# Symb0x76/ChineseChessZero

Hardware: NVIDIA B200
Metric: self-play moves/sec at 400 playouts (higher is better)
Workload: dtype bf16

## Files before the change

### chinesechesszero_b200/_lib.py

```python
from __future__ import annotations

import ctypes
import os

import numpy as np
import torch

from . import build as _build

BOARD_BYTES = 96
MAX_MOVES = 128
N_ACTIONS = 2086
PLANE_ELEMS = 10710
KEY_WINDOW = 128

FLAG_CHECK, FLAG_NOMOVES, FLAG_INSUFFICIENT, FLAG_FOURFOLD, FLAG_SIXTY = 1, 2, 4, 8, 16
FLAG_TIE_MASK = FLAG_INSUFFICIENT | FLAG_FOURFOLD | FLAG_SIXTY
STATUS_EXPAND_FAILED, STATUS_TREE_DROPPED = 1, 2
STATUS_NODE_OVERFLOW = STATUS_EXPAND_FAILED
ADVANCE_NEW_GAME, ADVANCE_DROP_TREE, ADVANCE_KEEP = -1, -2, -3
CTL_HEAD, CTL_TAIL, CTL_EXPAND_FAILED, CTL_TREES_DROPPED, CTL_MIN_FREE, CTL_WORDS = 0, 1, 2, 3, 4, 8
NODE_BYTES = 24
MAX_CHILDREN = 119
POLICY_PROBS, POLICY_LOGITS = 0, 1
CONV_VARIANT_1CTA, CONV_VARIANT_PAIR, CONV_VARIANT_2PAIRS, CONV_VARIANT_4PAIRS = 1, 2, 2 | 32, 2 | 64

EXPORTS = (
    "ccz_version", "ccz_last_error", "ccz_init", "ccz_action_table", "ccz_set_order_policy", "ccz_get_order_policy",
    "ccz_boards_start",
    "ccz_movegen_encode", "ccz_board_keys_init", "ccz_board_push", "ccz_mcts_pool_init", "ccz_mcts_reset",
    "ccz_mcts_reserve", "ccz_mcts_migrate", "ccz_mcts_select",
    "ccz_mcts_expand_backup", "ccz_mcts_root_visits", "ccz_mcts_advance", "ccz_replay_pack", "ccz_conv3x3_c256", "ccz_conv3x3_plan", "ccz_stem_lookup",
    "ccz_heads_pack",
)


class CczError(RuntimeError):
    pass


class ArenaStruct(ctypes.Structure):

    _fields_ = [
        ("n_games", ctypes.c_int32),
        ("n_pages", ctypes.c_int32),
        ("page_shift", ctypes.c_int32),
        ("max_pages", ctypes.c_int32),
        ("d_nodes", ctypes.c_void_p),
        ("d_links", ctypes.c_void_p),
        ("d_free_ring", ctypes.c_void_p),
        ("d_pool_ctl", ctypes.c_void_p),
        ("d_page_list", ctypes.c_void_p),
        ("d_page_fill", ctypes.c_void_p),
        ("d_n_pages", ctypes.c_void_p),
        ("d_n_pages_new", ctypes.c_void_p),
        ("d_list_sel", ctypes.c_void_p),
        ("d_alloc_page", ctypes.c_void_p),
        ("d_alloc_off", ctypes.c_void_p),
        ("d_root", ctypes.c_void_p),
        ("d_n_nodes", ctypes.c_void_p),
        ("d_status", ctypes.c_void_p),
        ("d_root_boards", ctypes.c_void_p),
        ("d_root_keys", ctypes.c_void_p),
    ]


# ... 15 lines not shown
        except Exception as e:
            if not os.path.exists(path):
                raise CczError(f"building {path} failed ({e}); there is no CPU fallback") from e
    if not os.path.exists(path):
        raise CczError(
            f"{path} is missing: run `python -c 'import __graft_entry__ as g; g.build()'` "
            "(nvcc -gencode arch=compute_100a,code=sm_100a); there is no CPU fallback"
        )
    lib = ctypes.CDLL(path)
    vp, i32, f32 = ctypes.c_void_p, ctypes.c_int, ctypes.c_float
    lib.ccz_version.restype = i32
    lib.ccz_last_error.restype = ctypes.c_char_p
    lib.ccz_init.restype = i32
    lib.ccz_action_table.argtypes = [vp, vp, vp]
    lib.ccz_boards_start.argtypes = [vp, i32, vp]
    lib.ccz_set_order_policy.argtypes = [vp]
    lib.ccz_get_order_policy.argtypes = [vp]
    lib.ccz_movegen_encode.argtypes = [vp, i32, vp, vp, vp, vp, vp]
    lib.ccz_board_keys_init.argtypes = [vp, i32, vp, vp]
    lib.ccz_board_push.argtypes = [vp, vp, i32, vp, vp]
    lib.ccz_mcts_pool_init.argtypes = [ctypes.POINTER(ArenaStruct), vp]
    lib.ccz_mcts_reset.argtypes = [ctypes.POINTER(ArenaStruct), vp, vp]
    lib.ccz_mcts_reserve.argtypes = [ctypes.POINTER(ArenaStruct), i32, vp]
    lib.ccz_mcts_migrate.argtypes = [ctypes.POINTER(ArenaStruct), ctypes.POINTER(ArenaStruct), vp]
    lib.ccz_mcts_select.argtypes = [ctypes.POINTER(ArenaStruct), f32, vp, vp, vp]
    lib.ccz_mcts_expand_backup.argtypes = [ctypes.POINTER(ArenaStruct), vp, vp, i32, vp, vp, vp, vp, vp]
    lib.ccz_mcts_root_visits.argtypes = [ctypes.POINTER(ArenaStruct), vp, vp, vp, vp]
    lib.ccz_mcts_advance.argtypes = [ctypes.POINTER(ArenaStruct), vp, vp]
    lib.ccz_replay_pack.argtypes = [vp, vp, vp, vp, vp, i32, vp, vp, vp]
    lib.ccz_conv3x3_c256.argtypes = [vp, vp, vp, vp, vp, i32, i32, vp]
    lib.ccz_stem_lookup.argtypes = [vp, i32, vp, vp, vp, vp]
    lib.ccz_conv3x3_plan.argtypes = [i32, i32, i32, vp]
    lib.ccz_heads_pack.argtypes = [vp, i32, vp, i32, i32, vp]
    for name in EXPORTS:
        if name not in ("ccz_last_error",):
            getattr(lib, name).restype = i32
    _lib = lib
    pinned = os.path.join(os.path.dirname(os.path.abspath(__file__)), "order_policy.json")
    if os.path.exists(pinned):
        import json

        with open(pinned) as f:
            set_order_policy(json.load(f))
    return lib


def check(rc: int, what: str) -> None:
    if rc != 0:
        msg = load().ccz_last_error().decode("utf-8", "replace")
        raise CczError(f"{what} failed ({rc}): {msg}")


def stream_ptr(device=None) -> int:
    return torch.cuda.current_stream(device).cuda_stream


def _ptr(t: torch.Tensor | None) -> int | None:
    if t is None:
        return None
    if not t.is_cuda:
        raise CczError("device tensor expected (the C ABI takes device pointers)")
    if not t.is_contiguous():
        raise CczError("contiguous tensor expected")
    return t.data_ptr()


# ... 240 lines not shown
                                    out.data_ptr(), int(x.shape[0]), int(variant), stream_ptr(x.device)),
            "ccz_conv3x3_c256",
        )
    return out


def stem_lookup(boards: torch.Tensor, table: torch.Tensor, bias_turn: torch.Tensor, out: torch.Tensor | None = None) -> torch.Tensor:
    n = boards.shape[0]
    if boards.dtype != torch.uint8 or boards.shape[1:] != (BOARD_BYTES,):
        raise CczError("stem_lookup: boards must be uint8 (n,96)")
    if table.dtype != torch.bfloat16 or tuple(table.shape) != (9, 16, 256) or bias_turn.dtype != torch.float32 \
            or tuple(bias_turn.shape) != (2, 9, 256):
        raise CczError("stem_lookup: table must be bf16 (9,16,256) and bias_turn fp32 (2,9,256)")
    if out is None:
        out = torch.empty((n, 256, 10, 9), dtype=torch.bfloat16, device=boards.device).contiguous(memory_format=torch.channels_last)
    elif tuple(out.shape) != (n, 256, 10, 9) or out.dtype != torch.bfloat16 or not out.is_contiguous(memory_format=torch.channels_last):
        raise CczError("stem_lookup: out must be bf16 (n,256,10,9) channels_last")
    with torch.cuda.device(boards.device):
        check(load().ccz_stem_lookup(_ptr(boards), n, _ptr(table), _ptr(bias_turn), out.data_ptr(), stream_ptr(boards.device)),
              "ccz_stem_lookup")
    return out


def heads_pack(h: torch.Tensor, operands: torch.Tensor, value_off: int) -> torch.Tensor:
    n = operands.shape[0]
    if h.dtype != torch.bfloat16 or operands.dtype != torch.bfloat16 or tuple(h.shape) != (n * 90, 32):
        raise CczError("heads_pack: h must be bf16 (n*90, 32) and operands bf16 (n, K)")
    with torch.cuda.device(h.device):
        check(load().ccz_heads_pack(_ptr(h), n, _ptr(operands), int(operands.shape[1]), int(value_off), stream_ptr(h.device)),
              "ccz_heads_pack")
    return operands


def conv3x3_plan(n_boards: int, variant: int = 0, resident_clusters: int = 74) -> dict:
    out = (ctypes.c_int32 * 6)()
    check(load().ccz_conv3x3_plan(int(n_boards), int(variant), int(resident_clusters), out), "ccz_conv3x3_plan")
    keys = ("rows_per_tile", "n_tiles", "n_items", "n_full", "split_log2", "clusters")
    return dict(zip(keys, (int(v) for v in out)))
```

### chinesechesszero_b200/csrc/ccz_b200.cu

```cuda
#include "../../include/ccz_b200.h"

#include <cuda_runtime.h>

#include <cstdio>
#include <cstdlib>
#include <cstring>
#include <utility>
#include <string>

#include "ccz_movegen.cuh"
#include "ccz_mcts.cuh"
#include "ccz_replay.cuh"
#include "ccz_conv.cuh"
#include "ccz_stem.cuh"
#include "ccz_heads.cuh"

#ifndef CCZ_CONV_DEFAULT_PAIRS
#define CCZ_CONV_DEFAULT_PAIRS 1
#endif

namespace {

thread_local std::string g_err;

// ... 439 lines not shown
            return fail(-3, "ccz_conv3x3_c256: cuTensorMapEncodeTiled(skip) failed");
    } else {
        ts = ty;
    }
    cudaError_t e;
#define CCZ_CONV_LAUNCH(CG, PAIRS)                                                                                      \
    (d_skip ? cv::launch_variant<CG, PAIRS, true>(tx, tw, ts, ty, d_bias, n_tiles, tail_split, dbg, s)     \
            : cv::launch_variant<CG, PAIRS, false>(tx, tw, ts, ty, d_bias, n_tiles, tail_split, dbg, s))
    if (cta_group == 1) e = CCZ_CONV_LAUNCH(1, 1);
    else if (pairs == 1) e = CCZ_CONV_LAUNCH(2, 1);
    else if (pairs == 2) e = CCZ_CONV_LAUNCH(2, 2);
    else e = CCZ_CONV_LAUNCH(2, 4);
#undef CCZ_CONV_LAUNCH
    if (e != cudaSuccess) return fail(-2, "conv3x3_c256_kernel launch", e);
    return 0;
}

int ccz_conv3x3_plan(int n_boards, int variant, int resident_clusters, int32_t *out) {
    namespace cv = ccz::conv;
    if (n_boards <= 0 || resident_clusters <= 0 || !out || variant < 0 || variant >= 128)
        return fail(-1, "ccz_conv3x3_plan: bad argument");
    int cta_group = variant & 3, pairs = 1 << ((variant >> 5) & 3);
    if (variant == 0) { cta_group = 2; pairs = CCZ_CONV_DEFAULT_PAIRS; }
    if (cta_group == 0) cta_group = 2;
    if (cta_group == 3 || pairs > 4 || (cta_group == 1 && pairs != 1)) return fail(-1, "ccz_conv3x3_plan: unsupported variant");
    const long long m = (long long)n_boards * cv::BOARD_HW;
    const int rows_per_tile = cv::BM * cta_group * pairs;
    const int n_tiles = (int)((m + rows_per_tile - 1) / rows_per_tile);
    const cv::Plan pl = cv::plan_items(n_tiles, resident_clusters, !(variant & 4));
    out[0] = rows_per_tile; out[1] = n_tiles; out[2] = pl.n_items; out[3] = pl.n_full; out[4] = pl.split_log2; out[5] = pl.clusters;
    return 0;
}

int ccz_stem_lookup(const uint8_t *d_boards, int n, const void *d_table, const float *d_bias_turn, void *d_y, ccz_stream_t s) {
    namespace st = ccz::stem;
    if (n < 0) return fail(-1, "ccz_stem_lookup: n < 0");
    if (n == 0) return 0;
    if (!d_boards || !d_table || !d_bias_turn || !d_y) return fail(-1, "ccz_stem_lookup: NULL pointer");
    if (((uintptr_t)d_boards & 3) || (((uintptr_t)d_table | (uintptr_t)d_bias_turn | (uintptr_t)d_y) & 15))
        return fail(-1, "ccz_stem_lookup: pointers must be 16-byte aligned (boards 4-byte)");
    static int n_sm_dev[64] = {0};
    int dev = 0;
    CCZ_CUDA(cudaGetDevice(&dev));
    if (dev < 0 || dev >= 64) return fail(-1, "ccz_stem_lookup: device index out of range");
    int &n_sm = n_sm_dev[dev];
    if (!n_sm) {
        CCZ_CUDA(cudaDeviceGetAttribute(&n_sm, cudaDevAttrMultiProcessorCount, dev));
        CCZ_CUDA(cudaFuncSetAttribute(st::stem_lookup_kernel, cudaFuncAttributeMaxDynamicSharedMemorySize, st::SMEM_BYTES));
    }
    int blocks = 2 * n_sm;
    const int need = (n + st::WARPS - 1) / st::WARPS;
    if (blocks > need) blocks = need;
    st::stem_lookup_kernel<<<blocks, st::WARPS * 32, st::SMEM_BYTES, s>>>(d_boards, n, static_cast<const uint4 *>(d_table),
                                                                         reinterpret_cast<const float4 *>(d_bias_turn),
                                                                         static_cast<uint4 *>(d_y));
    return check_launch("stem_lookup_kernel");
}

int ccz_heads_pack(const void *d_h, int n, void *d_operands, int row_elems, int value_off, ccz_stream_t s) {
    namespace hd = ccz::heads;
    if (n < 0) return fail(-1, "ccz_heads_pack: n < 0");
    if (n == 0) return 0;
    if (!d_h || !d_operands) return fail(-1, "ccz_heads_pack: NULL pointer");
    if (((uintptr_t)d_h & 15) || ((uintptr_t)d_operands & 3)) return fail(-1, "ccz_heads_pack: h must be 16-byte, operands 4-byte aligned");
    if ((row_elems & 1) || (value_off & 1) || value_off < hd::N_POLICY * hd::HW || row_elems < value_off + hd::N_VALUE * hd::HW)
        return fail(-1, "ccz_heads_pack: operand row must hold 1530 policy + 630 value elements at even offsets");
// ... 7 lines not shown
```

### chinesechesszero_b200/csrc/ccz_conv.cuh

```cuda
#pragma once

#include <cuda.h>
#include <cuda_bf16.h>
#include <cuda_runtime.h>

#include <cstdint>

#ifndef CCZ_CONV_BACKOFF_NS
#define CCZ_CONV_BACKOFF_NS 256
#endif

namespace ccz {
namespace conv {

constexpr int C = 256;
constexpr int BOARD_H = 10, BOARD_W = 9, BOARD_HW = 90;
constexpr int BM = 128;
constexpr int BN = 256;
constexpr int BK = 64;
constexpr int KBLOCKS = 9 * (C / BK);
constexpr int UMMA_K = 16;
constexpr int THREADS = 256;

template <int CG>
// ... 385 lines not shown
                    o.z = pack_bf16x2(fmaxf(f[4], 0.f), fmaxf(f[5], 0.f));
                    o.w = pack_bf16x2(fmaxf(f[6], 0.f), fmaxf(f[7], 0.f));
                    *cell = o;
                }
            }
            tc_fence_before();
            __syncwarp();
            if (lane == 0) {
                if constexpr (CG == 2) mbar_arrive_cluster(tempty0 + 8 * acc); else mbar_arrive(bar_tempty + 8 * acc);
            }
            if (++acc == 2) { acc = 0; acc_phase ^= 1; }
            fence_proxy_async();
            asm volatile("bar.sync 1, 128;" ::: "memory");
            if (threadIdx.x == 128) {
                for (int g = 0; g < wi.n_w / 64; ++g) tma_store_2d(&tm_y, staging + g * (BM * 128), wi.n_off + g * 64, m0);
                tma_store_commit();
                tma_store_wait_read();
                if (HAS_SKIP) mbar_arrive(bar_stfree);
            }
            asm volatile("bar.sync 1, 128;" ::: "memory");
        }
        if (threadIdx.x == 128) tma_store_wait_all();
    }

    __syncwarp();
    tc_fence_before();
    if constexpr (CLUSTER > 1) cluster_sync_all(); else __syncthreads();
    if (warp == 2) {
        tc_fence_after();
        tmem_dealloc<CG>(tmem_base, 512);
    }
}

typedef CUresult (*EncodeTiledFn)(CUtensorMap *, CUtensorMapDataType, cuuint32_t, void *, const cuuint64_t *, const cuuint64_t *,
                                  const cuuint32_t *, const cuuint32_t *, CUtensorMapInterleave, CUtensorMapSwizzle, CUtensorMapL2promotion,
                                  CUtensorMapFloatOOBfill);
typedef CUresult (*EncodeIm2colFn)(CUtensorMap *, CUtensorMapDataType, cuuint32_t, void *, const cuuint64_t *, const cuuint64_t *, const int *,
                                   const int *, cuuint32_t, cuuint32_t, const cuuint32_t *, CUtensorMapInterleave, CUtensorMapSwizzle,
                                   CUtensorMapL2promotion, CUtensorMapFloatOOBfill);

struct Driver {
    EncodeTiledFn tiled = nullptr;
    EncodeIm2colFn im2col = nullptr;
    bool ready = false;
};

inline const char *driver_init(Driver &d) {
    if (d.ready) return nullptr;
    cudaDriverEntryPointQueryResult q;
    void *f = nullptr;
    if (cudaGetDriverEntryPoint("cuTensorMapEncodeTiled", &f, cudaEnableDefault, &q) != cudaSuccess || q != cudaDriverEntryPointSuccess || !f)
        return "cuTensorMapEncodeTiled not available from the driver";
    d.tiled = reinterpret_cast<EncodeTiledFn>(f);
    f = nullptr;
    if (cudaGetDriverEntryPoint("cuTensorMapEncodeIm2col", &f, cudaEnableDefault, &q) != cudaSuccess || q != cudaDriverEntryPointSuccess || !f)
        return "cuTensorMapEncodeIm2col not available from the driver";
    d.im2col = reinterpret_cast<EncodeIm2colFn>(f);
    d.ready = true;
    return nullptr;
}

inline bool encode_rows(const Driver &d, CUtensorMap *m, const void *ptr, uint64_t rows, uint64_t cols, uint32_t box_rows) {
    const cuuint64_t dims[2] = {cols, rows};
    const cuuint64_t strides[1] = {cols * 2};
    const cuuint32_t box[2] = {64, box_rows};
    const cuuint32_t es[2] = {1, 1};
// ... 37 lines not shown
    int dev = 0, n_sm = 0;
    cudaError_t e0 = cudaGetDevice(&dev);
    if (e0 != cudaSuccess) return e0;
    if (dev < 0 || dev >= 64) return cudaErrorInvalidDevice;
    int &max_clusters = max_clusters_dev[dev];
    cudaLaunchConfig_t cfg = {};
    cfg.blockDim = dim3(THREADS);
    cfg.dynamicSmemBytes = Cfg<CG>::SMEM_BYTES;
    cfg.stream = stream;
    cudaLaunchAttribute at[1];
    at[0].id = cudaLaunchAttributeClusterDimension;
    at[0].val.clusterDim.x = CLUSTER;
    at[0].val.clusterDim.y = 1;
    at[0].val.clusterDim.z = 1;
    cfg.attrs = at;
    cfg.numAttrs = 1;
    if (!max_clusters) {
        cudaError_t e = cudaDeviceGetAttribute(&n_sm, cudaDevAttrMultiProcessorCount, dev);
        if (e != cudaSuccess) return e;
        e = cudaFuncSetAttribute(kern, cudaFuncAttributeMaxDynamicSharedMemorySize, Cfg<CG>::SMEM_BYTES);
        if (e != cudaSuccess) return e;
        cfg.gridDim = dim3((unsigned)(n_sm / CLUSTER * CLUSTER));
        int n = 0;
        e = cudaOccupancyMaxActiveClusters(&n, kern, &cfg);
        if (e != cudaSuccess) return e;
        if (n < 1) return cudaErrorInvalidConfiguration;
        max_clusters = n < n_sm / CLUSTER ? n : n_sm / CLUSTER;
    }
    const Plan pl = plan_items(n_tiles, max_clusters, tail_split != 0);
    cfg.gridDim = dim3((unsigned)(pl.clusters * CLUSTER));
    return cudaLaunchKernelEx(&cfg, kern, tx, tw, ts, ty, bias, pl.n_items, pl.n_full, pl.split_log2, dbg);
}

}
}
```

### chinesechesszero_b200/net.py

```python
from __future__ import annotations

import os

import numpy as np
import torch
import torch.nn.functional as F
from torch import nn

from . import _lib

PIECES = 7
PLAYS = 17
N_ACTIONS = _lib.N_ACTIONS
FLOP_PER_POSITION = 2 * 4_275_314_716


class ResBlock(nn.Module):

    def __init__(self, num_channels=256):
        super().__init__()
        self.conv1 = nn.Conv2d(num_channels, num_channels, kernel_size=(3, 3), stride=(1, 1), padding=1)
        self.conv1_bn = nn.BatchNorm2d(num_channels)
        self.conv1_act = nn.ReLU()
        self.conv2 = nn.Conv2d(num_channels, num_channels, kernel_size=(3, 3), stride=(1, 1), padding=1)
# ... 41 lines not shown


def _round_up(n: int, m: int) -> int:
    return (n + m - 1) // m * m


def _fold(conv: nn.Conv2d, bn: nn.BatchNorm2d):
    w = conv.weight.detach().float()
    b = conv.bias.detach().float() if conv.bias is not None else torch.zeros(w.shape[0], device=w.device)
    scale = bn.weight.detach().float() / torch.sqrt(bn.running_var.detach().float() + bn.eps)
    return w * scale.view(-1, 1, 1, 1), (b - bn.running_mean.detach().float()) * scale + bn.bias.detach().float()


def stem_tables(w: torch.Tensor, b: torch.Tensor):
    wf = w.float()
    co = wf.shape[0]
    table = torch.zeros((9, 16, co), dtype=torch.float32, device=w.device)
    for t in range(1, 8):
        table[:, t, :] = wf[:, 7 * PIECES + t - 1].reshape(co, 9).t()
        table[:, 8 + t, :] = wf[:, 15 * PIECES + t - 1].reshape(co, 9).t()
    turn_w = wf[:, 16 * PIECES:17 * PIECES].sum(1)
    bias_turn = torch.zeros((2, 9, co), dtype=torch.float32, device=w.device)
    for rc in range(3):
        for cc in range(3):
            rows = [r for r in range(3) if not (rc == 0 and r == 0) and not (rc == 2 and r == 2)]
            cols = [c for c in range(3) if not (cc == 0 and c == 0) and not (cc == 2 and c == 2)]
            bias_turn[0, rc * 3 + cc] = b.float()
            bias_turn[1, rc * 3 + cc] = b.float() + turn_w[:, rows][:, :, cols].sum((1, 2))
    return table.to(torch.bfloat16).contiguous(), bias_turn.contiguous()


class BatchedEvaluator:

    CONV_IMPLS = ("k9", "k9_skip", "cudnn", "torch")

    def __init__(self, net: Net, device="cuda", dtype=torch.bfloat16, fused_epilogue: bool = True,
                 conv_impl: str | None = None, chunk: int | None = None):
        self.device = torch.device(device)
        self.dtype = dtype
        self.chunk = int(os.environ.get("CCZ_EVAL_CHUNK", "0")) if chunk is None else int(chunk)
        if conv_impl is None:
            conv_impl = os.environ.get("CCZ_CONV_IMPL", "k9") if fused_epilogue else "torch"
        if conv_impl not in self.CONV_IMPLS:
            raise ValueError(f"conv_impl must be one of {self.CONV_IMPLS}")
        k9_ok = self.device.type == "cuda" and dtype == torch.bfloat16 and net.conv_block.out_channels == 256
        if conv_impl in ("k9", "k9_skip") and not k9_ok:
            conv_impl = "cudnn"
        self.conv_impl = conv_impl
        self.fused = conv_impl != "torch"
        self.n_evals = 0
        self.use_heads_pack = os.environ.get("CCZ_HEADS_PACK", "1") != "0"
        self.conv_events: list | None = None
        self.refresh(net)

    def _keep(self, key: str, t: torch.Tensor) -> torch.Tensor:
        old = self._params.get(key)
        if old is not None and old.shape == t.shape and old.dtype == t.dtype and old.stride() == t.stride():
            old.copy_(t)
            return old
        self._params[key] = t
        return t

    @torch.no_grad()
    def refresh(self, net: Net) -> None:
        dev, dt = self.device, self.dtype
        cl = torch.channels_last
        if not hasattr(self, "_params"):
            self._params: dict[str, torch.Tensor] = {}
            self.version = 0
        self.version += 1
        keep = self._keep

        def conv_params(key, conv, bn):
            w, b = _fold(conv, bn)
            return (keep(key + ".w", w.to(dev, dt).contiguous(memory_format=cl)), keep(key + ".b", b.to(dev, dt)),
                    keep(key + ".b32", b.to(dev, torch.float32).contiguous()))

        self.stem = conv_params("stem", net.conv_block, net.conv_block_bn)
        if self.conv_impl in ("k9", "k9_skip"):
            table, bias_turn = stem_tables(self.stem[0], self.stem[2])
            self.stem_lookup = (keep("stem.table", table), keep("stem.bias_turn", bias_turn))
        else:
            self.stem_lookup = None
        self.blocks = [(conv_params(f"rb{i}.1", rb.conv1, rb.conv1_bn), conv_params(f"rb{i}.2", rb.conv2, rb.conv2_bn))
                       for i, rb in enumerate(net.res_blocks)]
        pw, pb = _fold(net.policy_conv, net.policy_bn)
        vw, vb = _fold(net.value_conv, net.value_bn)
        self.heads_w = keep("heads.w", torch.cat([pw, vw], 0).to(dev, dt).contiguous(memory_format=cl))
        self.heads_b = keep("heads.b", torch.cat([pb, vb], 0).to(dev, dt))
        self.policy_fc = (keep("pfc.w", net.policy_fc.weight.detach().to(dev, dt).clone()),
                          keep("pfc.b", net.policy_fc.bias.detach().to(dev, torch.float32).clone()))
        self.value_fc1 = (keep("vfc1.w", net.value_fc1.weight.detach().to(dev, dt).clone()),
                          keep("vfc1.b", net.value_fc1.bias.detach().to(dev, dt).clone()))
        self._kp, self._kv, self._np = _round_up(PLAYS * 90, 8), _round_up(PIECES * 90, 8), _round_up(N_ACTIONS, 8)
        wp = torch.zeros((self._np, self._kp), dtype=dt, device=dev)
        wp[:N_ACTIONS, :PLAYS * 90] = self.policy_fc[0]
        wv = torch.zeros((self.value_fc1[0].shape[0], self._kv), dtype=dt, device=dev)
        wv[:, :PIECES * 90] = self.value_fc1[0]
        self._fc_pad = (keep("pfc.pad", wp), keep("vfc1.pad", wv))
        if not hasattr(self, "_head_buf"):
            self._head_buf = {}
        hw = torch.zeros((32, self.heads_w.shape[1]), dtype=dt, device=dev)
        hw[:PLAYS + PIECES] = self.heads_w.reshape(PLAYS + PIECES, -1)
        hb = torch.zeros((32,), dtype=dt, device=dev)
        hb[:PLAYS + PIECES] = self.heads_b
        self._heads_gemm = (keep("heads.gemm_w", hw), keep("heads.gemm_b", hb))
        self.value_fc2 = (keep("vfc2.w", net.value_fc2.weight.detach().to(dev, torch.float32).clone()),
                          keep("vfc2.b", net.value_fc2.bias.detach().to(dev, torch.float32).clone()))

    def _k9(self, x, w, b32, skip, out):
        if self.conv_events is None:
            return _lib.conv3x3_c256(x, w, b32, skip=skip, out=out)
        e0, e1 = torch.cuda.Event(enable_timing=True), torch.cuda.Event(enable_timing=True)
        e0.record()
        y = _lib.conv3x3_c256(x, w, b32, skip=skip, out=out)
        e1.record()
        self.conv_events.append((skip is not None, e0, e1))
        return y

    def _conv_relu(self, x, wb, k9=False):
        w, b, b32 = wb
        if k9:
            return self._k9(x, w, b32, None, None)
        if self.fused:
            return torch.cudnn_convolution_relu(x, w, b, (1, 1), (1, 1), (1, 1), 1)
        return F.relu_(F.conv2d(x, w, b, padding=1))

    def _conv_add_relu(self, x, wb, skip, k9=False):
        w, b, b32 = wb
        if k9:
            return self._k9(x, w, b32, skip, skip)
        if self.fused:
            return torch.cudnn_convolution_add_relu(x, w, skip, 1.0, b, (1, 1), (1, 1), (1, 1), 1)
        return F.relu_(F.conv2d(x, w, b, padding=1).add_(skip))

    @property
    def needs_planes(self) -> bool:
        return self.stem_lookup is None

    @torch.no_grad()
    def forward(self, planes: torch.Tensor | None, boards: torch.Tensor | None = None):
        use_boards = boards is not None and self.stem_lookup is not None
        g = boards.shape[0] if use_boards else planes.shape[0]
        if self.chunk and g > self.chunk:
            parts = [self._forward(None if use_boards else planes[i:i + self.chunk],
                                   boards[i:i + self.chunk] if use_boards else None) for i in range(0, g, self.chunk)]
            return torch.cat([p[0] for p in parts]), torch.cat([p[1] for p in parts])
        return self._forward(None if use_boards else planes, boards if use_boards else None)

    def _forward(self, planes, boards=None):
        if boards is not None:
            g = boards.shape[0]
            x = _lib.stem_lookup(boards, *self.stem_lookup)
        else:
            g = planes.shape[0]
            x = planes.view(g, PLAYS * PIECES, 10, 9).contiguous(memory_format=torch.channels_last)
            x = self._conv_relu(x, self.stem)
        k9_plain, k9_skip = self.conv_impl == "k9", self.conv_impl in ("k9", "k9_skip")
        for c1, c2 in self.blocks:
            y = self._conv_relu(x, c1, k9_plain)
            x = self._conv_add_relu(y, c2, x, k9_skip)
        if self.device.type == "cuda":
            rows = x.permute(0, 2, 3, 1).reshape(g * 90, x.shape[1])
            h = F.linear(rows, *self._heads_gemm)
            buf = self._head_buf.get(g)
            if buf is None:
                buf = self._head_buf[g] = torch.zeros((g, self._kp + self._kv), dtype=h.dtype, device=h.device)
                if len(self._head_buf) > 8:
                    self._head_buf.pop(next(iter(self._head_buf)))
            if self.dtype == torch.bfloat16 and self.use_heads_pack:
                _lib.heads_pack(h, buf, self._kp)
            else:
                h = F.relu_(h).view(g, 90, 32)
                buf[:, :PLAYS * 90].view(g, PLAYS, 90).copy_(h[:, :, :PLAYS].transpose(1, 2))
                buf[:, self._kp:self._kp + PIECES * 90].view(g, PIECES, 90).copy_(h[:, :, PLAYS:PLAYS + PIECES].transpose(1, 2))
            logits = F.linear(buf[:, :self._kp], self._fc_pad[0])[:, :N_ACTIONS].float() + self.policy_fc[1]
            v = F.relu_(F.linear(buf[:, self._kp:], self._fc_pad[1], self.value_fc1[1])).float()
        else:
            h = F.relu_(F.conv2d(x, self.heads_w, self.heads_b))
            hp = h[:, :PLAYS].reshape(g, PLAYS * 90)
            hv = h[:, PLAYS:].reshape(g, PIECES * 90)
            logits = F.linear(hp, self.policy_fc[0]).float() + self.policy_fc[1]
            v = F.relu_(F.linear(hv, *self.value_fc1)).float()
        v = torch.tanh(F.linear(v, *self.value_fc2)).view(g)
        return logits, v

    def __call__(self, planes, leaf_boards=None):
        logits, v = self.forward(planes, leaf_boards)
        self.n_evals += logits.shape[0]
        return logits, _lib.POLICY_LOGITS, v


class PolicyValueNet:

# ... 40 lines not shown
```

### include/ccz_b200.h

```cpp
#ifndef CCZ_B200_H
#define CCZ_B200_H

#include <stdint.h>

#ifdef __cplusplus
extern "C" {
#endif

typedef struct CUstream_st *ccz_stream_t;

#define CCZ_BOARD_BYTES 96
#define CCZ_MAX_MOVES 128
#define CCZ_N_ACTIONS 2086
#define CCZ_PLANE_ELEMS 10710
#define CCZ_KEY_WINDOW 128

#define CCZ_FLAG_CHECK 1
#define CCZ_FLAG_NOMOVES 2
#define CCZ_FLAG_INSUFFICIENT 4
#define CCZ_FLAG_FOURFOLD 8
#define CCZ_FLAG_SIXTY 16
#define CCZ_FLAG_TIE_MASK (CCZ_FLAG_INSUFFICIENT | CCZ_FLAG_FOURFOLD | CCZ_FLAG_SIXTY)

#define CCZ_STATUS_EXPAND_FAILED 1
// ... 79 lines not shown
int ccz_board_keys_init(const uint8_t *d_boards, int n, uint64_t *d_keys, ccz_stream_t s);

int ccz_mcts_pool_init(const ccz_arena *a, ccz_stream_t s);

int ccz_mcts_reset(const ccz_arena *a, const uint8_t *d_mask , ccz_stream_t s);

int ccz_mcts_reserve(const ccz_arena *a, int pages_per_game, ccz_stream_t s);

int ccz_mcts_migrate(const ccz_arena *src, const ccz_arena *dst, ccz_stream_t s);

int ccz_mcts_select(const ccz_arena *a, float c_puct, uint8_t *d_leaf_boards ,
                    int32_t *d_leaf_nodes , ccz_stream_t s);

int ccz_mcts_expand_backup(const ccz_arena *a, const int32_t *d_leaf_nodes, const float *d_policy,
                           int policy_kind, const float *d_values ,
                           const int16_t *d_move_ids, const int16_t *d_counts,
                           const uint8_t *d_flags, ccz_stream_t s);

int ccz_mcts_root_visits(const ccz_arena *a, int16_t *d_acts ,
                         int32_t *d_visits , int16_t *d_counts , ccz_stream_t s);

int ccz_mcts_advance(const ccz_arena *a, const int16_t *d_chosen, ccz_stream_t s);

int ccz_replay_pack(const uint8_t *d_hist_boards ,
                    const uint8_t *d_turn_plane , const int16_t *d_acts ,
                    const double *d_probs , const int16_t *d_counts, int n,
                    void *d_states_f16 , double *d_pi , ccz_stream_t s);

int ccz_conv3x3_c256(const void *d_x, const void *d_w, const float *d_bias, const void *d_skip, void *d_y,
                     int n_boards, int variant, ccz_stream_t s);

int ccz_conv3x3_plan(int n_boards, int variant, int resident_clusters, int32_t *out);

int ccz_stem_lookup(const uint8_t *d_boards, int n, const void *d_table, const float *d_bias_turn, void *d_y,
                    ccz_stream_t s);

int ccz_heads_pack(const void *d_h, int n, void *d_operands, int row_elems, int value_off, ccz_stream_t s);

#ifdef __cplusplus
}
#endif
#endif
```

Measured before the change: 372.7.

## Fuse entire residual conv tower into one persistent dataflow kernel

Adds a persistent 2-CTA cluster kernel that runs all residual 3x3 conv layers in a single launch. A work ring hands out (layer, tile) items grouped by L2-sized board groups, and per-tile done counters with acquire/release handle cross-layer halo dependencies. It also ping-pongs preallocated activation buffers, and the default 'k9' path now routes through this tower. The aim is to remove per-layer launch overhead and inter-layer bubbles and to keep activations L2-resident. The cost is spin-waiting on dependencies and the risk of deadlock or serialization if scheduling is poor.

```diff
diff --git a/chinesechesszero_b200/_lib.py b/chinesechesszero_b200/_lib.py
--- a/chinesechesszero_b200/_lib.py
+++ b/chinesechesszero_b200/_lib.py
@@ -31,7 +31,7 @@
     "ccz_movegen_encode", "ccz_board_keys_init", "ccz_board_push", "ccz_mcts_pool_init", "ccz_mcts_reset",
     "ccz_mcts_reserve", "ccz_mcts_migrate", "ccz_mcts_select",
     "ccz_mcts_expand_backup", "ccz_mcts_root_visits", "ccz_mcts_advance", "ccz_replay_pack", "ccz_conv3x3_c256", "ccz_conv3x3_plan", "ccz_stem_lookup",
-    "ccz_heads_pack",
+    "ccz_heads_pack", "ccz_conv_tower", "ccz_conv_tower_plan",
 )
 
 
@@ -113,6 +113,8 @@
     lib.ccz_stem_lookup.argtypes = [vp, i32, vp, vp, vp, vp]
     lib.ccz_conv3x3_plan.argtypes = [i32, i32, i32, vp]
     lib.ccz_heads_pack.argtypes = [vp, i32, vp, i32, i32, vp]
+    lib.ccz_conv_tower.argtypes = [vp, vp, vp, vp, i32, i32, i32, vp, vp]
+    lib.ccz_conv_tower_plan.argtypes = [i32, i32, i32, i32, vp]
     for name in EXPORTS:
         if name not in ("ccz_last_error",):
             getattr(lib, name).restype = i32
@@ -419,6 +421,44 @@
     return operands
 
 
+def conv_tower_work_ints(n_boards: int) -> int:
+    return 1 + (n_boards * 90 + 255) // 256
+
+
+def conv_tower(x: torch.Tensor, y: torch.Tensor, w: torch.Tensor, bias: torch.Tensor, work: torch.Tensor,
+               group_boards: int = 0) -> torch.Tensor:
+    cl = torch.channels_last
+    n, n_layers = int(x.shape[0]), int(w.shape[0])
+    if x.dtype != torch.bfloat16 or y.dtype != torch.bfloat16 or w.dtype != torch.bfloat16 or bias.dtype != torch.float32:
+        raise CczError("conv_tower: x, y, w must be bfloat16, bias float32")
+    if tuple(x.shape[1:]) != (256, 10, 9) or y.shape != x.shape or not x.is_contiguous(memory_format=cl) \
+            or not y.is_contiguous(memory_format=cl):
+        raise CczError("conv_tower: x and y must be (n,256,10,9) channels_last")
+    if tuple(w.shape) != (n_layers, 256, 2304) or not w.is_contiguous() or tuple(bias.shape) != (n_layers, 256) \
+            or not bias.is_contiguous():
+        raise CczError("conv_tower: w must be contiguous (L,256,2304), bias (L,256)")
+    if work.dtype != torch.int32 or work.numel() < conv_tower_work_ints(n) or not work.is_contiguous():
+        raise CczError("conv_tower: work must be contiguous int32 with conv_tower_work_ints(n) elements")
+    if not all(t.is_cuda and t.device == x.device for t in (y, w, bias, work)):
+        raise CczError("conv_tower: all tensors must be on x's CUDA device")
+    with torch.cuda.device(x.device):
+        check(load().ccz_conv_tower(x.data_ptr(), y.data_ptr(), w.data_ptr(), bias.data_ptr(), n, n_layers, int(group_boards),
+                                    work.data_ptr(), stream_ptr(x.device)), "ccz_conv_tower")
+    return x
+
+
+def conv_tower_plan(n_boards: int, n_layers: int, group_boards: int = 0) -> list[tuple[int, int, int, int]]:
+    out = (ctypes.c_int32 * 4)()
+    lib = load()
+    n_items = lib.ccz_conv_tower_plan(int(n_boards), int(n_layers), int(group_boards), 0, out)
+    check(min(n_items, 0), "ccz_conv_tower_plan")
+    items = []
+    for i in range(n_items):
+        lib.ccz_conv_tower_plan(int(n_boards), int(n_layers), int(group_boards), i, out)
+        items.append(tuple(int(v) for v in out))
+    return items
+
+
 def conv3x3_plan(n_boards: int, variant: int = 0, resident_clusters: int = 74) -> dict:
     out = (ctypes.c_int32 * 6)()
     check(load().ccz_conv3x3_plan(int(n_boards), int(variant), int(resident_clusters), out), "ccz_conv3x3_plan")
diff --git a/chinesechesszero_b200/csrc/ccz_b200.cu b/chinesechesszero_b200/csrc/ccz_b200.cu
--- a/chinesechesszero_b200/csrc/ccz_b200.cu
+++ b/chinesechesszero_b200/csrc/ccz_b200.cu
@@ -495,6 +495,49 @@
     return 0;
 }
 
+int ccz_conv_tower(void *d_x, void *d_y, const void *d_w, const float *d_bias, int n_boards, int n_layers, int group_boards,
+                   int32_t *d_work, ccz_stream_t s) {
+    namespace cv = ccz::conv;
+    if (n_boards < 0 || n_layers < 0) return fail(-1, "ccz_conv_tower: n_boards / n_layers < 0");
+    if (n_boards == 0 || n_layers == 0) return 0;
+    if (!d_x || !d_y || !d_w || !d_bias || !d_work) return fail(-1, "ccz_conv_tower: NULL pointer");
+    if (d_x == d_y) return fail(-1, "ccz_conv_tower: x and y must be distinct buffers");
+    if (group_boards < 0 || group_boards % cv::GROUP_QUANTUM) return fail(-1, "ccz_conv_tower: group_boards must be a multiple of 128");
+    if (((uintptr_t)d_x | (uintptr_t)d_w | (uintptr_t)d_y | (uintptr_t)d_work) & 15)
+        return fail(-1, "ccz_conv_tower: pointers must be 16-byte aligned");
+    if ((long long)n_layers * cv::BN > 0x7fffffffll / 8) return fail(-1, "ccz_conv_tower: n_layers too large");
+    if (group_boards == 0) {
+        int dev = 0, l2 = 0;
+        CCZ_CUDA(cudaGetDevice(&dev));
+        CCZ_CUDA(cudaDeviceGetAttribute(&l2, cudaDevAttrL2CacheSize, dev));
+        group_boards = cv::tower_default_group(l2);
+    }
+    static cv::Driver drv;
+    if (const char *err = cv::driver_init(drv)) return fail(-3, err);
+    const cv::TowerPlan plan = cv::tower_plan(n_boards, n_layers, group_boards);
+    const uint64_t m = (uint64_t)n_boards * cv::BOARD_HW;
+    CUtensorMap txi, tyi, txr, tyr, tw;
+    if (!cv::encode_im2col(drv, &txi, d_x, n_boards) || !cv::encode_im2col(drv, &tyi, d_y, n_boards))
+        return fail(-3, "ccz_conv_tower: cuTensorMapEncodeIm2col failed");
+    if (!cv::encode_rows(drv, &txr, d_x, m, cv::C, cv::BM) || !cv::encode_rows(drv, &tyr, d_y, m, cv::C, cv::BM) ||
+        !cv::encode_rows(drv, &tw, d_w, (uint64_t)n_layers * cv::BN, 9 * cv::C, (uint32_t)(cv::BN / 2)))
+        return fail(-3, "ccz_conv_tower: cuTensorMapEncodeTiled failed");
+    const cudaError_t e = cv::launch_tower(txi, tyi, txr, tyr, tw, d_bias, d_work, plan, s);
+    if (e != cudaSuccess) return fail(-2, "conv_tower_kernel launch", e);
+    return 0;
+}
+
+int ccz_conv_tower_plan(int n_boards, int n_layers, int group_boards, int item, int32_t *out) {
+    namespace cv = ccz::conv;
+    if (n_boards <= 0 || n_layers <= 0 || group_boards < 0 || group_boards % cv::GROUP_QUANTUM || !out)
+        return fail(-1, "ccz_conv_tower_plan: bad argument");
+    const cv::TowerPlan plan = cv::tower_plan(n_boards, n_layers, group_boards);
+    if (item < 0 || item >= plan.n_items) return fail(-1, "ccz_conv_tower_plan: item out of range");
+    const cv::TowerItem it = cv::tower_item(plan, item);
+    out[0] = it.layer; out[1] = it.tile; out[2] = it.dep_lo; out[3] = it.dep_hi;
+    return plan.n_items;
+}
+
 int ccz_stem_lookup(const uint8_t *d_boards, int n, const void *d_table, const float *d_bias_turn, void *d_y, ccz_stream_t s) {
     namespace st = ccz::stem;
     if (n < 0) return fail(-1, "ccz_stem_lookup: n < 0");
diff --git a/chinesechesszero_b200/csrc/ccz_conv.cuh b/chinesechesszero_b200/csrc/ccz_conv.cuh
--- a/chinesechesszero_b200/csrc/ccz_conv.cuh
+++ b/chinesechesszero_b200/csrc/ccz_conv.cuh
@@ -441,6 +441,317 @@
     }
 }
 
+struct TowerPlan {
+    int n_boards, n_layers, group_boards;
+    int group_tiles;
+    int n_groups;
+    int last_tiles;
+    int n_tiles, n_items;
+};
+struct TowerItem {
+    int layer, tile, dep_lo, dep_hi;
+};
+constexpr int TILE_PX = 2 * BM;
+constexpr int GROUP_QUANTUM = 128;
+__host__ __device__ inline int ceil_div(long long a, int b) { return (int)((a + b - 1) / b); }
+
+inline TowerPlan tower_plan(int n_boards, int n_layers, int group_boards) {
+    TowerPlan p;
+    if (group_boards <= 0 || group_boards >= n_boards) group_boards = ceil_div(n_boards, GROUP_QUANTUM) * GROUP_QUANTUM;
+    p.n_boards = n_boards;
+    p.n_layers = n_layers;
+    p.group_boards = group_boards;
+    p.group_tiles = group_boards * BOARD_HW / TILE_PX;
+    p.n_groups = ceil_div(n_boards, group_boards);
+    p.last_tiles = ceil_div((long long)(n_boards - (p.n_groups - 1) * group_boards) * BOARD_HW, TILE_PX);
+    p.n_tiles = (p.n_groups - 1) * p.group_tiles + p.last_tiles;
+    p.n_items = p.n_tiles * n_layers;
+    return p;
+}
+__host__ __device__ inline TowerItem tower_item(const TowerPlan &p, int item) {
+    const int per_full = p.n_layers * p.group_tiles;
+    int g = item / per_full, r = item - g * per_full, tiles = p.group_tiles;
+    if (g >= p.n_groups - 1) {
+        g = p.n_groups - 1;
+        r = item - g * per_full;
+        tiles = p.last_tiles;
+    }
+    TowerItem it;
+    it.layer = r / tiles;
+    const int t = r - it.layer * tiles, t0 = g * p.group_tiles;
+    it.tile = t0 + t;
+    it.dep_lo = it.layer ? t0 + (t > 0 ? t - 1 : 0) : 1;
+    it.dep_hi = it.layer ? t0 + (t + 1 < tiles ? t + 1 : tiles - 1) : 0;
+    return it;
+}
+
+constexpr int RING = 4;
+constexpr int RING_CONSUMERS = 7 + 6;
+
+__device__ __forceinline__ int ld_acquire_gpu(const int *p) {
+    int v;
+    asm volatile("ld.acquire.gpu.global.b32 %0, [%1];" : "=r"(v) : "l"(p) : "memory");
+    return v;
+}
+__device__ __forceinline__ void red_release_gpu_add(int *p, int v) {
+    asm volatile("red.release.gpu.global.add.s32 [%0], %1;" ::"l"(p), "r"(v) : "memory");
+}
+__device__ __forceinline__ void fence_proxy_async_global() { asm volatile("fence.proxy.async.global;" ::: "memory"); }
+__device__ __forceinline__ void st_shared_cluster(uint32_t cluster_addr, int v) {
+    asm volatile("st.shared::cluster.b32 [%0], %1;" ::"r"(cluster_addr), "r"(v) : "memory");
+}
+__device__ __forceinline__ int ld_shared_volatile(uint32_t addr) {
+    int v;
+    asm volatile("ld.volatile.shared.b32 %0, [%1];" : "=r"(v) : "r"(addr) : "memory");
+    return v;
+}
+
+__device__ __forceinline__ void tower_wait_deps(const int *done, const TowerItem &it) {
+    const int need = 2 * it.layer;
+    for (int t = it.dep_lo; t <= it.dep_hi; ++t)
+        while (ld_acquire_gpu(done + t) < need) __nanosleep(32);
+    fence_proxy_async_global();
+}
+
+struct RingReader {
+    uint32_t ring_items, ring_full, ring_empty_lead;
+    int k = 0;
+    __device__ __forceinline__ int next() {
+        const int slot = k % RING;
+        const uint32_t phase = (uint32_t)(k / RING) & 1u;
+        ++k;
+        mbar_wait_cluster(ring_full + 8 * slot, phase);
+        const int item = ld_shared_volatile(ring_items + 4 * slot);
+        mbar_arrive_cluster(ring_empty_lead + 8 * slot);
+        return item;
+    }
+};
+
+template <bool SKIP>
+__device__ __forceinline__ void epilogue_rows(uint32_t t_row, const float *bias_s, uint8_t *stg, int row) {
+#pragma unroll 1
+    for (int chunk = 0; chunk < BN / 32; ++chunk) {
+        uint32_t v[32];
+        tmem_ld32(t_row + chunk * 32, v);
+        tmem_ld_wait();
+        uint8_t *box_row = stg + (chunk >> 1) * (BM * 128) + row * 128;
+#pragma unroll
+        for (int j = 0; j < 4; ++j) {
+            const int c16 = (chunk & 1) * 4 + j;
+            uint4 *cell = reinterpret_cast<uint4 *>(box_row + ((c16 ^ (row & 7)) << 4));
+            const float4 b0 = *reinterpret_cast<const float4 *>(bias_s + chunk * 32 + j * 8);
+            const float4 b1 = *reinterpret_cast<const float4 *>(bias_s + chunk * 32 + j * 8 + 4);
+            float f[8] = {__uint_as_float(v[j * 8 + 0]) + b0.x, __uint_as_float(v[j * 8 + 1]) + b0.y,
+                          __uint_as_float(v[j * 8 + 2]) + b0.z, __uint_as_float(v[j * 8 + 3]) + b0.w,
+                          __uint_as_float(v[j * 8 + 4]) + b1.x, __uint_as_float(v[j * 8 + 5]) + b1.y,
+                          __uint_as_float(v[j * 8 + 6]) + b1.z, __uint_as_float(v[j * 8 + 7]) + b1.w};
+            if (SKIP) {
+                const uint4 sk = *cell;
+                const uint32_t w[4] = {sk.x, sk.y, sk.z, sk.w};
+#pragma unroll
+                for (int e = 0; e < 4; ++e) {
+                    f[2 * e] += __uint_as_float(w[e] << 16);
+                    f[2 * e + 1] += __uint_as_float(w[e] & 0xFFFF0000u);
+                }
+            }
+            uint4 o;
+            o.x = pack_bf16x2(fmaxf(f[0], 0.f), fmaxf(f[1], 0.f));
+            o.y = pack_bf16x2(fmaxf(f[2], 0.f), fmaxf(f[3], 0.f));
+            o.z = pack_bf16x2(fmaxf(f[4], 0.f), fmaxf(f[5], 0.f));
+            o.w = pack_bf16x2(fmaxf(f[6], 0.f), fmaxf(f[7], 0.f));
+            *cell = o;
+        }
+    }
+}
+
+__global__ void __launch_bounds__(THREADS, 1)
+conv_tower_kernel(const __grid_constant__ CUtensorMap tm_xi, const __grid_constant__ CUtensorMap tm_yi,
+                  const __grid_constant__ CUtensorMap tm_xr, const __grid_constant__ CUtensorMap tm_yr,
+                  const __grid_constant__ CUtensorMap tm_w, const float *__restrict__ bias, int *work, const TowerPlan plan) {
+    constexpr int CG = 2;
+    using K = Cfg<CG>;
+    extern __shared__ uint8_t smem_raw[];
+    const uint32_t smem_base = (smem_u32(smem_raw) + 1023u) & ~1023u;
+    const uint32_t a_smem = smem_base;
+    const uint32_t b_smem = a_smem + K::STAGES * K::A_BYTES;
+    const uint32_t staging = b_smem + K::STAGES * K::B_BYTES;
+    const uint32_t bias_smem = staging + K::STAGING_BYTES;
+    const uint32_t bars = bias_smem + K::BIAS_BYTES;
+    const uint32_t bar_full = bars;
+    const uint32_t bar_empty = bars + 8 * K::STAGES;
+    const uint32_t bar_tfull = bars + 16 * K::STAGES;
+    const uint32_t bar_tempty = bar_tfull + 16;
+    const uint32_t bar_skip = bar_tempty + 16;
+    const uint32_t bar_stfree = bar_skip + 8;
+    const uint32_t bar_ring_full = bar_stfree + 8;
+    const uint32_t bar_ring_empty = bar_ring_full + 8 * RING;
+    const uint32_t ring_items = bar_ring_empty + 8 * RING;
+    const uint32_t tmem_slot = ring_items + 4 * RING;
+    static_assert(16 * K::STAGES + 16 + 16 + 8 + 8 + 16 * RING + 4 * RING + 4 <= K::BAR_BYTES, "barrier area");
+    uint8_t *const smem_gen = smem_raw + (smem_base - smem_u32(smem_raw));
+    int *const done = work + 1;
+
+    const int warp = threadIdx.x >> 5, lane = threadIdx.x & 31;
+    const uint32_t prank = cluster_ctarank(), lead_rank = 0;
+
+    if (warp == 0 && lane == 0) {
+        tma_prefetch_desc(&tm_xi);
+        tma_prefetch_desc(&tm_yi);
+        tma_prefetch_desc(&tm_xr);
+        tma_prefetch_desc(&tm_yr);
+        tma_prefetch_desc(&tm_w);
+    }
+    if (warp == 1 && lane == 0) {
+        for (int i = 0; i < K::STAGES; ++i) {
+            mbar_init(bar_full + 8 * i, 1);
+            mbar_init(bar_empty + 8 * i, 1);
+        }
+        for (int i = 0; i < 2; ++i) {
+            mbar_init(bar_tfull + 8 * i, 1);
+            mbar_init(bar_tempty + 8 * i, 4 * CG);
+        }
+        mbar_init(bar_skip, 1);
+        mbar_init(bar_stfree, 1);
+        for (int i = 0; i < RING; ++i) {
+            mbar_init(bar_ring_full + 8 * i, 1);
+            mbar_init(bar_ring_empty + 8 * i, RING_CONSUMERS);
+        }
+        asm volatile("fence.mbarrier_init.release.cluster;" ::: "memory");
+    }
+    if (warp == 2) tmem_alloc<CG>(tmem_slot, 512);
+    tc_fence_before();
+    cluster_sync_all();
+    tc_fence_after();
+    const uint32_t tmem_base = *reinterpret_cast<volatile uint32_t *>(smem_gen + (tmem_slot - smem_base));
+    RingReader ring{ring_items, bar_ring_full, mapa(bar_ring_empty, lead_rank)};
+
+    if (warp == 0) {
+        if (lane == 0) {
+            const uint32_t full0 = mapa(bar_full, lead_rank);
+            int stage = 0;
+            uint32_t phase = 0;
+            for (int item; (item = ring.next()) >= 0;) {
+                const TowerItem it = tower_item(plan, item);
+                const CUtensorMap *tm_in = (it.layer & 1) ? &tm_yi : &tm_xi;
+                const int m0 = (it.tile * CG + (int)prank) * BM;
+                const int b_row = it.layer * BN + (int)prank * K::B_ROWS;
+                const int img = m0 / BOARD_HW, rem = m0 - img * BOARD_HW;
+                const int p = rem / BOARD_W, q = rem - p * BOARD_W;
+                tower_wait_deps(done, it);
+                for (int kb = 0; kb < KBLOCKS; ++kb) {
+                    const int tap = kb >> 2, c0 = (kb & 3) * BK;
+                    const int r = tap / 3, s = tap - 3 * r;
+                    mbar_wait(bar_empty + 8 * stage, phase ^ 1);
+                    if (prank == 0) mbar_expect_tx(bar_full + 8 * stage, CG * (K::A_BYTES + K::B_BYTES));
+                    tma_load_im2col<CG>(a_smem + stage * K::A_BYTES, tm_in, full0 + 8 * stage, c0, q - 1, p - 1, img, (uint16_t)s, (uint16_t)r);
+                    tma_load_2d<CG>(b_smem + stage * K::B_BYTES, &tm_w, full0 + 8 * stage, kb * BK, b_row);
+                    if (++stage == K::STAGES) { stage = 0; phase ^= 1; }
+                }
+            }
+        }
+    } else if (warp == 1) {
+        if (prank == 0 && lane == 0) {
+            constexpr uint32_t idesc = umma_idesc(BM * CG, BN);
+            int stage = 0;
+            uint32_t phase = 0, acc = 0, acc_phase = 0;
+            while (ring.next() >= 0) {
+                mbar_wait_cluster(bar_tempty + 8 * acc, acc_phase ^ 1);
+                tc_fence_after();
+                const uint32_t d_tmem = tmem_base + acc * BN;
+                for (int kb = 0; kb < KBLOCKS; ++kb) {
+                    mbar_wait(bar_full + 8 * stage, phase);
+                    tc_fence_after();
+                    const uint64_t a_desc = umma_desc_sw128(a_smem + stage * K::A_BYTES);
+                    const uint64_t b_desc = umma_desc_sw128(b_smem + stage * K::B_BYTES);
+#pragma unroll
+                    for (int k = 0; k < BK / UMMA_K; ++k)
+                        umma_bf16<CG>(d_tmem, a_desc + 2 * k, b_desc + 2 * k, idesc, (uint32_t)((kb | k) != 0));
+                    umma_commit<CG>(bar_empty + 8 * stage, 3);
+                    if (++stage == K::STAGES) { stage = 0; phase ^= 1; }
+                }
+                umma_commit<CG>(bar_tfull + 8 * acc, 3);
+                if (++acc == 2) { acc = 0; acc_phase ^= 1; }
+            }
+        }
+    } else if (warp == 2) {
+        if (prank == 0 && lane == 0) {
+            const uint32_t peer_items = mapa(ring_items, 1), peer_full = mapa(bar_ring_full, 1);
+            for (int k = 0;; ++k) {
+                const int slot = k % RING;
+                mbar_wait_cluster(bar_ring_empty + 8 * slot, ((uint32_t)(k / RING) & 1u) ^ 1u);
+                int item = atomicAdd(work, 1);
+                if (item >= plan.n_items) item = -1;
+                st_shared_cluster(mapa(ring_items, 0) + 4 * slot, item);
+                st_shared_cluster(peer_items + 4 * slot, item);
+                mbar_arrive_cluster(mapa(bar_ring_full, 0) + 8 * slot);
+                mbar_arrive_cluster(peer_full + 8 * slot);
+                if (item < 0) break;
+            }
+        }
+    } else if (warp == 3) {
+        if (lane == 0) {
+            for (int item; (item = ring.next()) >= 0;) {
+                const TowerItem it = tower_item(plan, item);
+                mbar_wait_relaxed(bar_stfree, (uint32_t)((ring.k - 1) & 1) ^ 1u);
+                if (it.layer & 1) {
+                    const int m0 = (it.tile * CG + (int)prank) * BM;
+                    tower_wait_deps(done, TowerItem{it.layer, it.tile, it.tile, it.tile});
+                    mbar_expect_tx(bar_skip, (BN / 64) * (BM * 128));
+                    for (int g = 0; g < BN / 64; ++g) tma_load_2d<1>(staging + g * (BM * 128), &tm_xr, bar_skip, g * 64, m0);
+                }
+            }
+        }
+    } else {
+        const int quarter = warp - 4, row = quarter * 32 + lane;
+        const uint32_t tempty0 = mapa(bar_tempty, lead_rank);
+        float *bias_s = reinterpret_cast<float *>(smem_gen + (bias_smem - smem_base));
+        uint8_t *stg = smem_gen + (staging - smem_base);
+        uint32_t acc = 0, acc_phase = 0, skip_it = 0;
+        for (;;) {
+            int item = 0;
+            if (lane == 0) item = ring.next();
+            item = __shfl_sync(0xffffffffu, item, 0);
+            if (item < 0) break;
+            const TowerItem it = tower_item(plan, item);
+            const int m0 = (it.tile * CG + (int)prank) * BM;
+            const int t = threadIdx.x - 128;
+            bias_s[t] = bias[it.layer * BN + t];
+            bias_s[t + 128] = bias[it.layer * BN + t + 128];
+            asm volatile("bar.sync 1, 128;" ::: "memory");
+            if (it.layer & 1) mbar_wait_relaxed(bar_skip, (skip_it++) & 1);
+            mbar_wait_relaxed(bar_tfull + 8 * acc, acc_phase);
+            tc_fence_after();
+            const uint32_t t_row = tmem_base + ((uint32_t)(quarter * 32) << 16) + acc * BN;
+            if (it.layer & 1) epilogue_rows<true>(t_row, bias_s, stg, row);
+            else epilogue_rows<false>(t_row, bias_s, stg, row);
+            tc_fence_before();
+            __syncwarp();
+            if (lane == 0) mbar_arrive_cluster(tempty0 + 8 * acc);
+            if (++acc == 2) { acc = 0; acc_phase ^= 1; }
+            fence_proxy_async();
+            asm volatile("bar.sync 1, 128;" ::: "memory");
+            if (threadIdx.x == 128) {
+                const CUtensorMap *tm_out = (it.layer & 1) ? &tm_xr : &tm_yr;
+                for (int g = 0; g < BN / 64; ++g) tma_store_2d(tm_out, staging + g * (BM * 128), g * 64, m0);
+                tma_store_commit();
+                tma_store_wait_all();
+                fence_proxy_async_global();
+                red_release_gpu_add(done + it.tile, 1);
+                mbar_arrive(bar_stfree);
+            }
+            asm volatile("bar.sync 1, 128;" ::: "memory");
+        }
+    }
+
+    __syncwarp();
+    tc_fence_before();
+    cluster_sync_all();
+    if (warp == 2) {
+        tc_fence_after();
+        tmem_dealloc<CG>(tmem_base, 512);
+    }
+}
+
 typedef CUresult (*EncodeTiledFn)(CUtensorMap *, CUtensorMapDataType, cuuint32_t, void *, const cuuint64_t *, const cuuint64_t *,
                                   const cuuint32_t *, const cuuint32_t *, CUtensorMapInterleave, CUtensorMapSwizzle, CUtensorMapL2promotion,
                                   CUtensorMapFloatOOBfill);
@@ -544,5 +855,50 @@
     return cudaLaunchKernelEx(&cfg, kern, tx, tw, ts, ty, bias, pl.n_items, pl.n_full, pl.split_log2, dbg);
 }
 
-}
-}
+inline int tower_default_group(int l2_bytes) {
+    const long long per_quantum = 2ll * GROUP_QUANTUM * BOARD_HW * C * 2;
+    const long long q = (3ll * l2_bytes / 4) / per_quantum;
+    return (int)(q > 1 ? q : 1) * GROUP_QUANTUM;
+}
+
+inline cudaError_t launch_tower(const CUtensorMap &txi, const CUtensorMap &tyi, const CUtensorMap &txr, const CUtensorMap &tyr,
+                                const CUtensorMap &tw, const float *bias, int *work, const TowerPlan &plan, cudaStream_t stream) {
+    static int max_clusters_dev[64] = {0};
+    int dev = 0;
+    cudaError_t e = cudaGetDevice(&dev);
+    if (e != cudaSuccess) return e;
+    if (dev < 0 || dev >= 64) return cudaErrorInvalidDevice;
+    int &max_clusters = max_clusters_dev[dev];
+    cudaLaunchConfig_t cfg = {};
+    cfg.blockDim = dim3(THREADS);
+    cfg.dynamicSmemBytes = Cfg<2>::SMEM_BYTES;
+    cfg.stream = stream;
+    cudaLaunchAttribute at[1];
+    at[0].id = cudaLaunchAttributeClusterDimension;
+    at[0].val.clusterDim.x = 2;
+    at[0].val.clusterDim.y = 1;
+    at[0].val.clusterDim.z = 1;
+    cfg.attrs = at;
+    cfg.numAttrs = 1;
+    if (!max_clusters) {
+        int n_sm = 0;
+        e = cudaDeviceGetAttribute(&n_sm, cudaDevAttrMultiProcessorCount, dev);
+        if (e != cudaSuccess) return e;
+        e = cudaFuncSetAttribute(conv_tower_kernel, cudaFuncAttributeMaxDynamicSharedMemorySize, Cfg<2>::SMEM_BYTES);
+        if (e != cudaSuccess) return e;
+        cfg.gridDim = dim3((unsigned)(n_sm / 2 * 2));
+        int n = 0;
+        e = cudaOccupancyMaxActiveClusters(&n, conv_tower_kernel, &cfg);
+        if (e != cudaSuccess) return e;
+        if (n < 1) return cudaErrorInvalidConfiguration;
+        max_clusters = n < n_sm / 2 ? n : n_sm / 2;
+    }
+    e = cudaMemsetAsync(work, 0, sizeof(int) * (size_t)(1 + plan.n_tiles), stream);
+    if (e != cudaSuccess) return e;
+    const int clusters = max_clusters < plan.n_items ? max_clusters : plan.n_items;
+    cfg.gridDim = dim3((unsigned)(clusters * 2));
+    return cudaLaunchKernelEx(&cfg, conv_tower_kernel, txi, tyi, txr, tyr, tw, bias, work, plan);
+}
+
+}
+}
diff --git a/chinesechesszero_b200/net.py b/chinesechesszero_b200/net.py
--- a/chinesechesszero_b200/net.py
+++ b/chinesechesszero_b200/net.py
@@ -97,7 +97,8 @@
 
 class BatchedEvaluator:
 
-    CONV_IMPLS = ("k9", "k9_skip", "cudnn", "torch")
+    CONV_IMPLS = ("k9", "k9_layers", "k9_skip", "cudnn", "torch")
+    K9_IMPLS = ("k9", "k9_layers", "k9_skip")
 
     def __init__(self, net: Net, device="cuda", dtype=torch.bfloat16, fused_epilogue: bool = True,
                  conv_impl: str | None = None, chunk: int | None = None):
@@ -109,13 +110,15 @@
         if conv_impl not in self.CONV_IMPLS:
             raise ValueError(f"conv_impl must be one of {self.CONV_IMPLS}")
         k9_ok = self.device.type == "cuda" and dtype == torch.bfloat16 and net.conv_block.out_channels == 256
-        if conv_impl in ("k9", "k9_skip") and not k9_ok:
+        if conv_impl in self.K9_IMPLS and not k9_ok:
             conv_impl = "cudnn"
         self.conv_impl = conv_impl
         self.fused = conv_impl != "torch"
         self.n_evals = 0
         self.use_heads_pack = os.environ.get("CCZ_HEADS_PACK", "1") != "0"
         self.conv_events: list | None = None
+        self.tower_group = 0
+        self._act_buf: dict[int, tuple] = {}
         self.refresh(net)
 
     def _keep(self, key: str, t: torch.Tensor) -> torch.Tensor:
@@ -142,7 +145,21 @@
                     keep(key + ".b32", b.to(dev, torch.float32).contiguous()))
 
         self.stem = conv_params("stem", net.conv_block, net.conv_block_bn)
-        if self.conv_impl in ("k9", "k9_skip"):
+        k9 = self.conv_impl in self.K9_IMPLS
+        if k9:
+            n_layers = 2 * len(net.res_blocks)
+            tw = self._params.get("tower.w")
+            if tw is None or tw.shape[0] != n_layers:
+                tw = self._params["tower.w"] = torch.empty((n_layers, 256, 9 * 256), dtype=dt, device=dev)
+                tb = self._params["tower.b32"] = torch.empty((n_layers, 256), dtype=torch.float32, device=dev)
+                wv = tw.view(n_layers, 256, 3, 3, 256).permute(0, 1, 4, 2, 3)
+                for i in range(n_layers):
+                    self._params[f"rb{i // 2}.{i % 2 + 1}.w"] = wv[i]
+                    self._params[f"rb{i // 2}.{i % 2 + 1}.b32"] = tb[i]
+            self.tower = (tw, self._params["tower.b32"])
+        else:
+            self.tower = None
+        if k9:
             table, bias_turn = stem_tables(self.stem[0], self.stem[2])
             self.stem_lookup = (keep("stem.table", table), keep("stem.bias_turn", bias_turn))
         else:
@@ -183,10 +200,10 @@
         self.conv_events.append((skip is not None, e0, e1))
         return y
 
-    def _conv_relu(self, x, wb, k9=False):
+    def _conv_relu(self, x, wb, k9=False, out=None):
         w, b, b32 = wb
         if k9:
-            return self._k9(x, w, b32, None, None)
+            return self._k9(x, w, b32, None, out)
         if self.fused:
             return torch.cudnn_convolution_relu(x, w, b, (1, 1), (1, 1), (1, 1), 1)
         return F.relu_(F.conv2d(x, w, b, padding=1))
@@ -198,6 +215,16 @@
         if self.fused:
             return torch.cudnn_convolution_add_relu(x, w, skip, 1.0, b, (1, 1), (1, 1), (1, 1), 1)
         return F.relu_(F.conv2d(x, w, b, padding=1).add_(skip))
+
+    def _acts(self, g: int):
+        buf = self._act_buf.get(g)
+        if buf is None:
+            x = torch.empty((g, 256, 10, 9), dtype=self.dtype, device=self.device).contiguous(memory_format=torch.channels_last)
+            buf = self._act_buf[g] = (x, torch.empty_like(x), torch.empty((_lib.conv_tower_work_ints(g),), dtype=torch.int32,
+                                                                         device=self.device))
+            if len(self._act_buf) > 8:
+                self._act_buf.pop(next(iter(self._act_buf)))
+        return buf
 
     @property
     def needs_planes(self) -> bool:
@@ -216,15 +243,20 @@
     def _forward(self, planes, boards=None):
         if boards is not None:
             g = boards.shape[0]
-            x = _lib.stem_lookup(boards, *self.stem_lookup)
+            x = _lib.stem_lookup(boards, *self.stem_lookup, out=self._acts(g)[0] if self.tower is not None else None)
         else:
             g = planes.shape[0]
             x = planes.view(g, PLAYS * PIECES, 10, 9).contiguous(memory_format=torch.channels_last)
             x = self._conv_relu(x, self.stem)
-        k9_plain, k9_skip = self.conv_impl == "k9", self.conv_impl in ("k9", "k9_skip")
-        for c1, c2 in self.blocks:
-            y = self._conv_relu(x, c1, k9_plain)
-            x = self._conv_add_relu(y, c2, x, k9_skip)
+        if self.conv_impl == "k9" and self.blocks:
+            _, y, work = self._acts(g)
+            x = _lib.conv_tower(x, y, *self.tower, work, self.tower_group)
+        else:
+            k9_plain, k9_skip = self.conv_impl == "k9_layers", self.conv_impl in self.K9_IMPLS
+            y = self._acts(g)[1] if k9_plain else None
+            for c1, c2 in self.blocks:
+                y = self._conv_relu(x, c1, k9_plain, out=y)
+                x = self._conv_add_relu(y, c2, x, k9_skip)
         if self.device.type == "cuda":
             rows = x.permute(0, 2, 3, 1).reshape(g * 90, x.shape[1])
             h = F.linear(rows, *self._heads_gemm)
diff --git a/include/ccz_b200.h b/include/ccz_b200.h
--- a/include/ccz_b200.h
+++ b/include/ccz_b200.h
@@ -135,6 +135,11 @@
 
 int ccz_conv3x3_plan(int n_boards, int variant, int resident_clusters, int32_t *out);
 
+int ccz_conv_tower(void *d_x, void *d_y, const void *d_w, const float *d_bias, int n_boards, int n_layers, int group_boards,
+                   int32_t *d_work, ccz_stream_t s);
+
+int ccz_conv_tower_plan(int n_boards, int n_layers, int group_boards, int item, int32_t *out);
+
 int ccz_stem_lookup(const uint8_t *d_boards, int n, const void *d_table, const float *d_bias_turn, void *d_y,
                     ccz_stream_t s);
 
```

Result: faster. 380.5 (median of 6 runs) (+2.1%).
